# Qi2019KB/UBPL-PoseEstimation

Hardware: AMD Instinct MI355X
Metric: images/sec training step (MT_UBPL, 2-stack HG, 256×256) at 1/2/4/8 GPUs; PCK@0.2 (higher is better)
Workload: dtype fp32; 1 GPU; MT_UBPL train step, 2 students + 2 EMA teachers, 2 views; model=StackedHourglass HG2 (K=16, AvgPool features), global_batch=32, per_gpu_batch=32, input=256x256x3, heatmap=16x64x64, parallelism=dp1

## Files before the change

### include/ubpl_hip.h

```cpp
#ifndef UBPL_HIP_H
#define UBPL_HIP_H
#include <stdint.h>

#ifdef __cplusplus
extern "C" {
#endif

int ubpl_render_heatmaps(const float* kps, float* hm, float* kps_out, int N, int K, int img_h, int img_w,
                         int inp_res, int out_res, float kernel_size, float sigma, float cutoff, void* stream);

int ubpl_heatmap_row_stats(const float* a, int64_t a_sb, int64_t a_ss, const float* t, int64_t t_sb, int64_t t_ss,
                           int64_t t_sm, int M, int B, int S, int K, int HW, float* sq_mean, float* amax,
                           float* tmax, void* stream);
int ubpl_loss_finalize(int kind, const float* sq_mean, const float* amax, const float* tmax, const float* gate,
                       const float* sw, int use_gate, int use_sw, int B, int S, int K, float thr, float* out_sum,
                       int* out_cnt, float* out_score, float* out_w, void* stream);
int ubpl_heatmap_row_grad(const float* a, int64_t a_sb, int64_t a_ss, const float* t, int64_t t_sb, int64_t t_ss,
                          int64_t t_sm, int M, int B, int S, int K, int HW, const float* w, const float* gscale,
                          float extra, float* da, int accumulate, void* stream);

int ubpl_fdl_cov_forward(const float* f1, const float* f2, const float* rowmask, int B, int S, int C, int HW,
                         float* cov, float* mu1, float* mu2, float* out_val, int* out_cnt, void* stream);
int ubpl_fdl_cov_backward(const float* f1, const float* f2, const float* rowmask, const float* cov, const float* mu1,
                          const float* mu2, const int* cnt, const float* gscale, int B, int S, int C, int HW,
// ... 142 lines not shown
int ubpl_upsample2x_add_forward_stats(const float* up, const float* low, int B, int C, int H, int W, float* out,
                                      float* part, void* stream);
int ubpl_bn_forward_stats_maxpool(const float* x, int B, int C, int H, int W, float* y, const float* gamma,
                                  const float* beta, float* rmean, float* rvar, float* mean_out, float* invstd_out,
                                  float* scale, float* shift, const float* pgamma, const float* pbeta, float* prmean,
                                  float* prvar, float* pmean_out, float* pinvstd_out, float* pscale, float* pshift,
                                  float eps, float momentum, double* part, void* stream);
int ubpl_upsample2x_add_forward_bnstats(const float* up, const float* low, int B, int C, int H, int W, float* out,
                                        const float* gamma, const float* beta, float eps, float momentum,
                                        float* rmean, float* rvar, double* part, float* mean_out, float* invstd_out,
                                        float* scale, float* shift, void* stream);
int ubpl_bn_backward_pool(const float* dz, const float* x, int B, int C, int H, int W, const float* gamma,
                          const float* mean, const float* invstd, const float* scale, const float* shift, int relu,
                          double* scratch, const float* part, float* coef, float* dgamma, float* dbeta,
                          const float* add1, const float* pool_dy, const float* add2, float* dx, void* stream);

int ubpl_image_mean_u8(const uint8_t* imgs, int N, int64_t n_per_image, float* out, void* stream);
int ubpl_augment_warp(const uint8_t* imgs, int H, int W, const int* src_idx, const float* mat, const float* noise,
                      const float* img_mean, const float* chan_mean, int V, int Ho, int Wo, float* out, void* stream);

int ubpl_augment_chain(const uint8_t* imgs, int H, int W, const int* geo, const float* cs, const float* noise,
                       const float* img_mean, const float* chan_mean, int V, int Hm, int Wm, float* inter, int Ho,
                       int Wo, float* out, void* stream);

int ubpl_occlude(float* out, int V, int H, int W, const float* bank, const int64_t* off, const int* hw,
                 const int* pastes, const int* view_first, const float* chan_mean, void* stream);

#ifdef __cplusplus
}
#endif
// ... 2 lines not shown
```

### ubpl-poseestimation_amd/csrc/bn_bwd.hip

```cpp
#include "bn.h"

namespace {

__device__ __forceinline__ float fp16_scale_for(float bound) {
    if (!(bound > 0.f) || !isfinite(bound)) return 1.f;
    int e;
    frexpf(bound, &e);
    e = min(max(14 - e, -60), 60);
    return ldexpf(1.f, e);
}

template <bool VEC, bool BOUND>
__global__ void __launch_bounds__(256) bwd_stats_kernel(const float* __restrict__ dz, const float* __restrict__ x,
                                                       int B, int C, int HW, int bper,
                                                       const float* __restrict__ scale,
                                                       const float* __restrict__ shift,
                                                       const float* __restrict__ mean, int relu,
                                                       double* __restrict__ part, unsigned* __restrict__ cnt,
                                                       BwdOut o) {
    __shared__ double red[16];
    __shared__ float redf[16];
    const int c = blockIdx.x, sp = blockIdx.y;
    const int b0 = sp * bper, b1 = min(B, b0 + bper);
    const float sc = scale[c], sh = shift[c], mu = mean[c];
    float s1 = 0.f, s2 = 0.f;
    float mg = 0.f, mx = 0.f;
    if (VEC) {
        const int hw4 = HW >> 2;
        const int n4 = (b1 - b0) * hw4;
        const float4* x4 = reinterpret_cast<const float4*>(x);
        const float4* d4 = reinterpret_cast<const float4*>(dz);
        auto acc1 = [&](float4 xv, float4 g) {
            if (relu) {
                g.x = fmaf(xv.x, sc, sh) > 0.f ? g.x : 0.f;
                g.y = fmaf(xv.y, sc, sh) > 0.f ? g.y : 0.f;
                g.z = fmaf(xv.z, sc, sh) > 0.f ? g.z : 0.f;
                g.w = fmaf(xv.w, sc, sh) > 0.f ? g.w : 0.f;
            }
            s1 += (g.x + g.y) + (g.z + g.w);
            s2 = fmaf(g.x, xv.x - mu, fmaf(g.y, xv.y - mu, fmaf(g.z, xv.z - mu, fmaf(g.w, xv.w - mu, s2))));
            if (BOUND) {
                mg = fmaxf(mg, fmaxf(fmaxf(fabsf(g.x), fabsf(g.y)), fmaxf(fabsf(g.z), fabsf(g.w))));
                mx = fmaxf(mx, fmaxf(fmaxf(fabsf(xv.x - mu), fabsf(xv.y - mu)),
                                     fmaxf(fabsf(xv.z - mu), fabsf(xv.w - mu))));
            }
        };
        auto off_of = [&](int i) {
            const int bb = i / hw4, o4 = i - bb * hw4;
            return ((int64_t)(b0 + bb) * C + c) * hw4 + o4;
        };
        const int st = blockDim.x;
        if (n4 <= 8 * st) {
            float4 xv[8], g[8];
#pragma unroll
            for (int u = 0; u < 8; ++u) {
                const int i = threadIdx.x + u * st;
                if (i < n4) {
                    const int64_t off = off_of(i);
                    xv[u] = x4[off];
                    g[u] = d4[off];
                }
            }
#pragma unroll
            for (int u = 0; u < 8; ++u)
                if (threadIdx.x + u * st < n4) acc1(xv[u], g[u]);
        } else {
            for (int i = threadIdx.x; i < n4; i += st) {
                const int64_t off = off_of(i);
                acc1(x4[off], d4[off]);
            }
        }
    } else {
        const int n = (b1 - b0) * HW;
        for (int i = threadIdx.x; i < n; i += blockDim.x) {
            const int bb = i / HW, o1 = i - bb * HW;
            const int64_t off = ((int64_t)(b0 + bb) * C + c) * HW + o1;
            const float xv = x[off];
            float g = dz[off];
            if (relu && !(fmaf(xv, sc, sh) > 0.f)) g = 0.f;
            s1 += g;
            s2 = fmaf(g, xv - mu, s2);
            if (BOUND) {
                mg = fmaxf(mg, fabsf(g));
                mx = fmaxf(mx, fabsf(xv - mu));
// ... 117 lines not shown

__device__ __forceinline__ void add_pool_grad(float4& v, float4 xv, int64_t off, PoolGeom g, float2 pd) {
    const float4 w = shfl_xor4(xv, 1 << g.lw4);
    const bool bot = (off >> g.lw4) & 1;
    const float4 t = bot ? w : xv, b = bot ? xv : w;
    int a0, a1;
    max4(t.x, t.y, b.x, b.y, a0);
    max4(t.z, t.w, b.z, b.w, a1);
    const int q = bot ? 2 : 0;
    v.x += a0 == q ? pd.x : 0.f;
    v.y += a0 == q + 1 ? pd.x : 0.f;
    v.z += a1 == q ? pd.y : 0.f;
    v.w += a1 == q + 1 ? pd.y : 0.f;
}

struct PoolGrad {
    const float* dy;
    PoolGeom g;
};

template <bool POOL>
__global__ void __launch_bounds__(256) bwd_apply_vec_kernel(const float* dz, const float* __restrict__ x, int C,
                                                           int HW4, int64_t total4, const float* __restrict__ scale,
                                                           const float* __restrict__ shift,
                                                           const float* __restrict__ mean, int relu,
                                                           const float* __restrict__ ca,
                                                           const float* __restrict__ cb,
                                                           const float* __restrict__ cc, const float* add1,
                                                           const float* add2, float* dx, PoolGrad p) {
    const int64_t stride = (int64_t)gridDim.x * blockDim.x;
    for (int64_t i = (int64_t)blockIdx.x * blockDim.x + threadIdx.x; i < total4; i += stride) {
        const int c = (int)((POOL ? i >> p.g.lhw4 : i / HW4) % C);
        const float sc = scale[c], sh = shift[c], mu = mean[c], a = ca[c], b = cb[c], cx = cc[c];
        const float4 xv = reinterpret_cast<const float4*>(x)[i];
        const float4 g = reinterpret_cast<const float4*>(dz)[i];
        float2 pd;
        if (POOL) pd = reinterpret_cast<const float2*>(p.dy)[half_index(i, p.g)];
        float4 v = bwd_one4(g, xv, sc, sh, mu, a, b, cx, relu);
        if (add1) add4(v, reinterpret_cast<const float4*>(add1)[i]);
        if (POOL) add_pool_grad(v, xv, i, p.g, pd);
        if (add2) add4(v, reinterpret_cast<const float4*>(add2)[i]);
        reinterpret_cast<float4*>(dx)[i] = v;
    }
}

template <bool POOL, int U>
__global__ void __launch_bounds__(256) bwd_apply_plane_kernel(const float* dz, const float* __restrict__ x, int C,
                                                             int HW4, const float* __restrict__ scale,
                                                             const float* __restrict__ shift,
                                                             const float* __restrict__ mean, int relu,
                                                             const float* __restrict__ ca,
                                                             const float* __restrict__ cb,
                                                             const float* __restrict__ cc, const float* add1,
                                                             const float* add2, float* dx, PoolGrad p) {
    const int pl = blockIdx.y;
    const int c = pl % C;
    const float sc = scale[c], sh = shift[c], mu = mean[c], a = ca[c], b = cb[c], cx = cc[c];
    const int64_t base = (int64_t)pl * HW4 + blockIdx.x * (256 * U) + threadIdx.x;
    const float4* x4 = reinterpret_cast<const float4*>(x) + base;
    const float4* d4 = reinterpret_cast<const float4*>(dz) + base;
    float4 xv[U], g[U], q1[U], q2[U];
    float2 pd[U];
#pragma unroll
    for (int u = 0; u < U; ++u) {
        xv[u] = x4[u * 256];
        g[u] = d4[u * 256];
        if (POOL) pd[u] = reinterpret_cast<const float2*>(p.dy)[half_index(base + u * 256, p.g)];
        if (add1) q1[u] = reinterpret_cast<const float4*>(add1)[base + u * 256];
        if (add2) q2[u] = reinterpret_cast<const float4*>(add2)[base + u * 256];
    }
#pragma unroll
    for (int u = 0; u < U; ++u) {
        float4 v = bwd_one4(g[u], xv[u], sc, sh, mu, a, b, cx, relu);
        if (add1) add4(v, q1[u]);
        if (POOL) add_pool_grad(v, xv[u], base + u * 256, p.g, pd[u]);
        if (add2) add4(v, q2[u]);
        reinterpret_cast<float4*>(dx)[base + u * 256] = v;
    }
}

__global__ void __launch_bounds__(256) bwd_apply_kernel(const float* dz, const float* __restrict__ x, int C, int HW,
                                                       int64_t total, const float* __restrict__ scale,
                                                       const float* __restrict__ shift,
                                                       const float* __restrict__ mean, int relu,
                                                       const float* __restrict__ ca, const float* __restrict__ cb,
                                                       const float* __restrict__ cc, const float* add1,
                                                       const float* add2, float* dx) {
    const int64_t stride = (int64_t)gridDim.x * blockDim.x;
    for (int64_t i = (int64_t)blockIdx.x * blockDim.x + threadIdx.x; i < total; i += stride) {
        const int c = (int)((i / HW) % C);
// ... 25 lines not shown
    const int64_t HW = (int64_t)H * W;
    const int64_t o = ((int64_t)b * C + 16 * g) * HW + (in ? h * W + w : 0);
    float v[16];
#pragma unroll
    for (int j = 0; j < 16; ++j) {
        const int c = 16 * g + j;
        const float r = bwd_one(dz[o + j * HW], x[o + j * HW], scale[c], shift[c], mean[c], ca[c], cb[c], cc[c], relu);
        v[j] = in ? r : 0.f;
    }
    ubpl::store_psa_row<NP>(v, dst + (((int64_t)(b * G + g) * Hp + hp) * Wp + wq) * 16, plane,
                            NP == 2 ? *dxscale : 1.f);
}

int bwd_stats(const float* dz, const float* x, int B, int C, int HW, const float* gamma, const float* mean,
              const float* invstd, const float* scale, const float* shift, int relu, double* scratch,
              const float* part, float* coef, float* dgamma, float* dbeta, hipStream_t st, bool bound = false) {
    BwdOut o{gamma, invstd, dgamma, dbeta, coef, coef + C, coef + 2 * C, nullptr, nullptr, nullptr};
    if (part != nullptr) {
        if (bound) return (int)hipErrorInvalidValue;
        const int64_t N = (int64_t)B * HW;
        hipLaunchKernelGGL(bn_bwd_finalize_kernel, dim3(C), dim3(FT), 0, st, part, (N + 63) / 64, N, o);
        UBPL_LAUNCH_CHECK();
        return 0;
    }
    if (C > MAXBN || scratch == nullptr) return (int)hipErrorInvalidValue;
    int bper, gs;
    stats_grid(B, C, HW, bper, gs);
    const Scratch s = carve(scratch);
    if (bound) {
        o.bnd = s.bnd;
        o.tcnt = s.tcnt;
        o.dxscale = coef + 3 * C;
    }
    const bool vec = (HW % 4 == 0) && ((((uintptr_t)dz | (uintptr_t)x) & 15) == 0);
    return pick(
        [&](auto VEC, auto BOUND) {
            hipLaunchKernelGGL((bwd_stats_kernel<VEC != 0, BOUND != 0>), dim3(C, gs), dim3(256), 0, st, dz, x, B, C,
                               HW, bper, scale, shift, mean, relu, s.slab, s.cnt, o);
            UBPL_LAUNCH_CHECK();
            return 0;
        },
        among<0, 1>{vec}, among<0, 1>{bound});
}

template <bool POOL>
int launch_apply4(const float* dz, const float* x, int B, int C, int HW, const float* scale, const float* shift,
                  const float* mean, int relu, const float* coef, const float* add1, const float* add2, float* dx,
                  PoolGrad p, hipStream_t st) {
    const float *ca = coef, *cb = coef + C, *cc = coef + 2 * C;
    const int hw4 = HW / 4;
    if (hw4 % 256 != 0 || (int64_t)B * C >= 65536) {
        const int64_t total4 = (int64_t)B * C * hw4;
        hipLaunchKernelGGL(bwd_apply_vec_kernel<POOL>, dim3(grid_ew(total4)), dim3(256), 0, st, dz, x, C, hw4, total4,
                           scale, shift, mean, relu, ca, cb, cc, add1, add2, dx, p);
        UBPL_LAUNCH_CHECK();
        return 0;
    }
    const int u = hw4 % 1024 == 0 ? 4 : (hw4 % 512 == 0 ? 2 : 1);
    return pick(
        [&](auto U) {
            hipLaunchKernelGGL((bwd_apply_plane_kernel<POOL, U>), dim3((unsigned)(hw4 / (256 * U)), (unsigned)(B * C)),
                               dim3(256), 0, st, dz, x, C, hw4, scale, shift, mean, relu, ca, cb, cc, add1, add2, dx,
                               p);
            UBPL_LAUNCH_CHECK();
            return 0;
        },
        among<4, 2, 1>{u});
}

}

UBPL_API int ubpl_bn_backward_partials(const float* dz, const float* x, int B, int C, int HW, const float* scale,
                                       const float* shift, const float* mean, int relu, float* part, void* stream) {
    const int64_t N = (int64_t)B * HW;
    const int64_t np = (N + 63) / 64;
    const bool vec = (HW % 4 == 0) && ((((uintptr_t)dz | (uintptr_t)x) & 15) == 0);
// ... 29 lines not shown
            return 0;
        },
        among<1, 2, 3>{npieces});
}

UBPL_API int ubpl_bn_backward(const float* dz, const float* x, int B, int C, int HW, const float* gamma,
                              const float* mean, const float* invstd, const float* scale, const float* shift,
                              int relu, double* scratch, const float* part, float* coef, float* dgamma,
                              float* dbeta, const float* add1, const float* add2, float* dx, void* stream) {
    hipStream_t st = (hipStream_t)stream;
    const int e = bwd_stats(dz, x, B, C, HW, gamma, mean, invstd, scale, shift, relu, scratch, part, coef, dgamma,
                            dbeta, st);
    if (e) return e;
    const uintptr_t al = (uintptr_t)dz | (uintptr_t)x | (uintptr_t)dx | (uintptr_t)add1 | (uintptr_t)add2;
    if (HW % 4 == 0 && (al & 15) == 0)
        return launch_apply4<false>(dz, x, B, C, HW, scale, shift, mean, relu, coef, add1, add2, dx, PoolGrad{}, st);
    const int64_t total = (int64_t)B * C * HW;
    hipLaunchKernelGGL(bwd_apply_kernel, dim3(grid_ew(total)), dim3(256), 0, st, dz, x, C, HW, total, scale, shift,
                       mean, relu, coef, coef + C, coef + 2 * C, add1, add2, dx);
    UBPL_LAUNCH_CHECK();
    return 0;
}

UBPL_API int ubpl_bn_backward_pool(const float* dz, const float* x, int B, int C, int H, int W, const float* gamma,
                                   const float* mean, const float* invstd, const float* scale, const float* shift,
                                   int relu, double* scratch, const float* part, float* coef, float* dgamma,
                                   float* dbeta, const float* add1, const float* pool_dy, const float* add2,
                                   float* dx, void* stream) {
    const int HW = H * W;
    if (pool_dy == nullptr)
        return ubpl_bn_backward(dz, x, B, C, HW, gamma, mean, invstd, scale, shift, relu, scratch, part, coef, dgamma,
                                dbeta, add1, add2, dx, stream);
    PoolGrad p{pool_dy, {}};
    const uintptr_t al = (uintptr_t)dz | (uintptr_t)x | (uintptr_t)dx | (uintptr_t)add1 | (uintptr_t)add2;
    if (B < 1 || C < 1 || !pool_geom(H, W, p.g) || (al & 15) || (((uintptr_t)pool_dy) & 7))
        return (int)hipErrorInvalidValue;
    hipStream_t st = (hipStream_t)stream;
    const int e = bwd_stats(dz, x, B, C, HW, gamma, mean, invstd, scale, shift, relu, scratch, part, coef, dgamma,
                            dbeta, st);
    if (e) return e;
    return launch_apply4<true>(dz, x, B, C, HW, scale, shift, mean, relu, coef, add1, add2, dx, p, st);
}
```

### ubpl-poseestimation_amd/csrc/pool.hip

```cpp
#include "common.h"

namespace {

int grid_ew(int64_t n) {
    int64_t g = (n + 255) / 256;
    if (g > 8192) g = 8192;
    if (g < 1) g = 1;
    return (int)g;
}

__device__ __forceinline__ void wave_bn_partial(float v, int64_t i0, int C, int P, int64_t np, float* part) {
    const float s = ubpl::wave_sum(v);
    const float d = v - s * (1.f / 64.f);
    const float m2 = ubpl::wave_sum(d * d);
    if ((threadIdx.x & 63) == 0) {
        const int64_t bc = i0 / P;
        const int c = (int)(bc % C);
        const int64_t q = ((bc / C) * P + (i0 - bc * P)) >> 6;
        part[((int64_t)c * np + q) * 2] = s;
        part[((int64_t)c * np + q) * 2 + 1] = m2;
    }
}

template <bool STATS>
// ... 57 lines not shown
__global__ void __launch_bounds__(256) avgpool_fwd_kernel(const float* __restrict__ x, int64_t planes, int H, int W,
                                                         float* __restrict__ y) {
    const int Ho = H >> 1, Wo = W >> 1;
    const int64_t total = planes * Ho * Wo;
    const int64_t stride = (int64_t)gridDim.x * blockDim.x;
    for (int64_t i = (int64_t)blockIdx.x * blockDim.x + threadIdx.x; i < total; i += stride) {
        const int ow = (int)(i % Wo);
        const int64_t t = i / Wo;
        const int oh = (int)(t % Ho);
        const int64_t pl = t / Ho;
        const float* p = x + (pl * H + 2 * oh) * W + 2 * ow;
        y[i] = (((p[0] + p[1]) + p[W]) + p[W + 1]) / 4.f;
    }
}

__global__ void __launch_bounds__(256) avgpool_bwd_kernel(const float* __restrict__ dy, int64_t planes, int H, int W,
                                                         float* __restrict__ dx, int accumulate) {
    const int Ho = H >> 1, Wo = W >> 1;
    const int64_t total = planes * Ho * Wo;
    const int64_t stride = (int64_t)gridDim.x * blockDim.x;
    for (int64_t i = (int64_t)blockIdx.x * blockDim.x + threadIdx.x; i < total; i += stride) {
        const int ow = (int)(i % Wo);
        const int64_t t = i / Wo;
        const int oh = (int)(t % Ho);
        const int64_t pl = t / Ho;
        const int64_t base = (pl * H + 2 * oh) * W + 2 * ow;
        const float g = dy[i] / 4.f;
        const int64_t offs[4] = {0, 1, W, W + 1};
#pragma unroll
        for (int q = 0; q < 4; ++q) {
// ... 71 lines not shown
            const float4 v = reinterpret_cast<const float4*>(x)[src];
            reinterpret_cast<float4*>(y)[i] = make_float4(v.w, v.z, v.y, v.x);
        } else {
            y[i] = x[src];
        }
    }
}

}

UBPL_API int ubpl_fliplr(const float* x, int64_t planes, int H, int W, float* y, void* stream) {
    if (planes < 0 || H < 0 || W < 0 || x == y) return (int)hipErrorInvalidValue;
    const int64_t rows = planes * H;
    if (rows == 0 || W == 0) return 0;
    if ((W % 4) == 0 && ((((uintptr_t)x) | ((uintptr_t)y)) & 15) == 0) {
        hipLaunchKernelGGL(fliplr_kernel<true>, dim3(grid_ew(rows * (W / 4))), dim3(256), 0, (hipStream_t)stream, x,
                           rows, W, y);
    } else {
        hipLaunchKernelGGL(fliplr_kernel<false>, dim3(grid_ew(rows * W)), dim3(256), 0, (hipStream_t)stream, x, rows,
                           W, y);
    }
    UBPL_LAUNCH_CHECK();
    return 0;
}

UBPL_API int ubpl_maxpool2x2_forward(const float* x, int64_t planes, int H, int W, float* y, void* stream) {
    const int64_t n = planes * (H / 2) * (W / 2);
    if (n == 0) return 0;
    hipLaunchKernelGGL(maxpool_fwd_kernel<false>, dim3(grid_ew(n)), dim3(256), 0, (hipStream_t)stream, x, planes, H,
                       W, y, 1, nullptr);
    UBPL_LAUNCH_CHECK();
    return 0;
}

UBPL_API int ubpl_maxpool2x2_forward_stats(const float* x, int B, int C, int H, int W, float* y, float* part,
                                           void* stream) {
    const int64_t planes = (int64_t)B * C;
    if (((H / 2) * (W / 2)) % 64 != 0 || part == nullptr) return (int)hipErrorInvalidValue;
    const int64_t n = planes * (H / 2) * (W / 2);
    if (n == 0) return 0;
    hipLaunchKernelGGL(maxpool_fwd_kernel<true>, dim3(grid_ew(n)), dim3(256), 0, (hipStream_t)stream, x, planes, H,
                       W, y, C, part);
    UBPL_LAUNCH_CHECK();
    return 0;
}

UBPL_API int ubpl_maxpool2x2_backward(const float* x, const float* dy, int64_t planes, int H, int W, float* dx,
                                      int accumulate, void* stream) {
    const int64_t n = planes * (H / 2) * (W / 2);
    if (n == 0) return 0;
    hipLaunchKernelGGL(maxpool_bwd_kernel, dim3(grid_ew(n)), dim3(256), 0, (hipStream_t)stream, x, dy, planes, H, W,
                       dx, accumulate);
    UBPL_LAUNCH_CHECK();
    return 0;
}

UBPL_API int ubpl_avgpool2x2_forward(const float* x, int64_t planes, int H, int W, float* y, void* stream) {
    const int64_t n = planes * (H / 2) * (W / 2);
    if (n == 0) return 0;
    hipLaunchKernelGGL(avgpool_fwd_kernel, dim3(grid_ew(n)), dim3(256), 0, (hipStream_t)stream, x, planes, H, W, y);
    UBPL_LAUNCH_CHECK();
    return 0;
}

UBPL_API int ubpl_avgpool2x2_backward(const float* dy, int64_t planes, int H, int W, float* dx, int accumulate,
                                      void* stream) {
    const int64_t n = planes * (H / 2) * (W / 2);
    if (n == 0) return 0;
    hipLaunchKernelGGL(avgpool_bwd_kernel, dim3(grid_ew(n)), dim3(256), 0, (hipStream_t)stream, dy, planes, H, W, dx,
                       accumulate);
    UBPL_LAUNCH_CHECK();
    return 0;
}

UBPL_API int ubpl_upsample2x_add_forward(const float* up, const float* low, int64_t planes, int H, int W, float* out,
                                         void* stream) {
    const int64_t n = planes * H * W;
    if (n == 0) return 0;
    if ((W % 4) == 0 && ((((uintptr_t)up) | ((uintptr_t)out)) & 15) == 0 && (((uintptr_t)low) & 7) == 0) {
        hipLaunchKernelGGL(upadd_fwd_vec_kernel, dim3(grid_ew(n / 4)), dim3(256), 0, (hipStream_t)stream, up, low, H,
                           W, n / 4, out);
        UBPL_LAUNCH_CHECK();
        return 0;
    }
    hipLaunchKernelGGL(upadd_fwd_kernel<false>, dim3(grid_ew(n)), dim3(256), 0, (hipStream_t)stream, up, low, planes,
                       H, W, out, 1, nullptr);
    UBPL_LAUNCH_CHECK();
    return 0;
}

UBPL_API int ubpl_upsample2x_add_forward_stats(const float* up, const float* low, int B, int C, int H, int W,
                                               float* out, float* part, void* stream) {
    const int64_t planes = (int64_t)B * C;
    if ((H * W) % 64 != 0 || part == nullptr) return (int)hipErrorInvalidValue;
    const int64_t n = planes * H * W;
    if (n == 0) return 0;
    hipLaunchKernelGGL(upadd_fwd_kernel<true>, dim3(grid_ew(n)), dim3(256), 0, (hipStream_t)stream, up, low, planes,
                       H, W, out, C, part);
    UBPL_LAUNCH_CHECK();
    return 0;
}

UBPL_API int ubpl_upsample2x_add_backward(const float* dout, int64_t planes, int H, int W, float* dlow,
                                          int accumulate, void* stream) {
    const int64_t n = planes * (H / 2) * (W / 2);
    if (n == 0) return 0;
    hipLaunchKernelGGL(upadd_bwd_kernel, dim3(grid_ew(n)), dim3(256), 0, (hipStream_t)stream, dout, planes, H, W, dlow,
                       accumulate);
    UBPL_LAUNCH_CHECK();
    return 0;
}

UBPL_API int ubpl_add(const float* a, const float* b, int64_t n, float* out, void* stream) {
    if (n == 0) return 0;
    hipLaunchKernelGGL(add_kernel, dim3(grid_ew(n)), dim3(256), 0, (hipStream_t)stream, a, b, n, out);
    UBPL_LAUNCH_CHECK();
    return 0;
}
```

### ubpl-poseestimation_amd/ubpl_amd/hourglass.py

```python
import math
import os

import torch
from torch import nn

from . import _lib
from . import kernels as Kn

BN_EPS = 1e-5
BN_MOMENTUM = 0.1
_PRODUCER_STATS = os.environ.get("UBPL_PRODUCER_STATS", "0") == "1"
_WGRAD3_64 = os.environ.get("UBPL_WGRAD3_64", "1") != "0"
_WGRAD1_SPLIT = os.environ.get("UBPL_WGRAD1_SPLIT", "1") != "0"
_BWD_EPI = os.environ.get("UBPL_BWD_EPI", "0") == "1"
_STEM_S2D = os.environ.get("UBPL_STEM_S2D", "1") != "0"
_STEM_WGRAD = os.environ.get("UBPL_STEM_WGRAD", "1") != "0"
_FWD_EPI = os.environ.get("UBPL_FWD_EPI", "0") == "1"
_FP16_BWD3 = os.environ.get("UBPL_FP16_BWD3", "1") != "0"
_UPADD_OOP = os.environ.get("UBPL_UPADD_OOP", "0") == "1"
_RELAYOUT_ONCE = os.environ.get("UBPL_RELAYOUT_ONCE", "0") == "1"
_SAVE_LOW3 = os.environ.get("UBPL_SAVE_LOW3", "")
_POOL_FUSE = 0 if (_PRODUCER_STATS or _FWD_EPI or _UPADD_OOP or _SAVE_LOW3) else \
    {"0": 0, "2": 2}.get(os.environ.get("UBPL_POOL_FUSE", "1"), 1)

# ... 410 lines not shown
        x1 = x
        if ex.fuse_ok(x1) and ex.fuse == 2:
            x = ex.bn_maxpool(None, x1, "pre.3.bn1")
            ex.give_coef(x, "pre.3.bn1")
        else:
            part = ex.stat_buffer((x1.shape[0], x1.shape[1], x1.shape[2] // 2, x1.shape[3] // 2))
            x = Kn.maxpool2x2(x1, stat_part=part)
            ex.give_part(x, part)
        ex.save("pre.2", x1)
        x = ex.residual("pre.3", x)
        x = ex.residual("pre.4", x)
        preds, feats = [], []
        for i in range(self.nStack):
            hg = ex.hourglass("hgs.%d.0" % i, 4, x, "features.%d.0.bn1" % i)
            f0 = ex.residual("features.%d.0" % i, hg)
            f = ex.conv_bn_relu("features.%d.1" % i, f0)
            if self.mode != "default" and not frozen:
                feats.append(Kn.avgpool2x2(f) if self.mode == "AvgPool" else Kn.maxpool2x2(f))
            pr = ex.conv("preds.%d.conv" % i, f)
            preds.append(pr)
            if i < self.nStack - 1:
                t = ex.conv("merge_preds.%d.conv.conv" % i, pr, res=x)
                x, part = ex.conv("merge_features.%d.conv.conv" % i, f, res=t, out=t, stats=True)
                ex.give_part(x, part)
            ex.save("stack.%d" % i, (f, pr))
        P = torch.stack(preds, 1)
        Fs = torch.stack(feats, 1) if feats else None
        return P, Fs, ex

    def _backward_impl(self, ex, dpreds, dfeats):
        ex.backward(dpreds, dfeats)


class _HourglassFn(torch.autograd.Function):
    @staticmethod
    def forward(ctx, imgs, anchor, model):
        preds, feats, ex = model._forward_impl(imgs, save=True)
        ctx.ex = ex
        ctx.model = model
        if feats is None:
# ... 144 lines not shown
    def stem(self, imgs):
        if self.ws.pieces in (1, 2, 3) and _STEM_S2D and Kn.stem_s2d_ok(imgs):
            np_ = Kn.backward_pieces(self.ws.pieces)
            ws = self.ws.stem_split(np_)
            xs = Kn.stem_s2d_split(imgs, 2, np_)
            y0 = Kn.conv2d_forward_psa(xs, ws, self.ws.P("pre.0.conv.bias"))
            if self.do_save and _STEM_WGRAD:
                self.saved_split["pre.0.conv"] = xs
        else:
            y0 = self.conv("pre.0.conv", imgs, stride=2)
        sc, sh = self.bn("pre.0.bn", y0)
        x0 = Kn.bn_apply(y0, sc, sh, relu=1)
        self.save("pre.0", (imgs, y0))
        return x0

    def conv_bn_relu(self, p, x):
        y, part = self.conv(p + ".conv", x, stats=True)
        sc, sh = self.bn(p + ".bn", y, part)
        f = Kn.bn_apply(y, sc, sh, relu=1)
        self.save(p, (x, y))
        return f

    def residual(self, p, x):
        cin = x.shape[1]
        cout = self.m._offs[p + ".conv3.conv.weight"][2][0]
        part = self.take_part(x)
        c1 = self.bnc(p + ".bn1")[:2] if self.take_coef(x, p + ".bn1") else self.bn(p + ".bn1", x, part)
        t1, part = self.conv(p + ".conv1.conv", x, pro=c1, stats=True)
        c2 = self.bn(p + ".bn2", t1, part)
        t2, part = self.conv(p + ".conv2.conv", t1, pro=c2, stats=True)
        c3 = self.bn(p + ".bn3", t2, part)
        if cin != cout:
            r = self.conv(p + ".skip_layer.conv", x)
            out, part = self.conv(p + ".conv3.conv", t2, pro=c3, res=r, out=r, stats=True)
        else:
            out, part = self.conv(p + ".conv3.conv", t2, pro=c3, res=x, stats=True)
# ... 34 lines not shown
        if _SAVE_LOW3 == "add":
            self.save(p + ".add_in", (up1.clone(), low3.clone()))
        out = Kn.upsample2x_add(up1, low3, out=up1, stat_part=part)
        if _SAVE_LOW3 == "add":
            self.save(p + ".add_out", out.clone())
        self.give_part(out, part)
        return out

    def _coef(self):
        return self.bcoef if self.bcoef is not None else self.m._ws[("coef", self.B)]

    def G(self, name):
        s, n, shp = self.m._offs[name]
        return self.gbuf[s:s + n].view(shp)

    def bn_bwd(self, name, dz, x, relu, add1=None, add2=None, out=None, part=None, pool_dy=None):
        sc, sh, mu, istd = self.bnc(name)
        if pool_dy is not None:
            return Kn.bn_backward_pool(dz, x, self.m.P(name + ".weight"), mu, istd, sc, sh, relu, self.bpart,
                                       self._coef(), self.G(name + ".weight"), self.G(name + ".bias"), add1=add1,
                                       pool_dy=pool_dy, add2=add2, out=out, part=part)
        return Kn.bn_backward(dz, x, self.m.P(name + ".weight"), mu, istd, sc, sh, relu, self.bpart, self._coef(),
                              self.G(name + ".weight"), self.G(name + ".bias"), add1=add1, add2=add2, out=out,
                              part=part)

    def bn_bwd_split(self, name, dz, x, relu, part=None, pieces=None, grads=True):
        sc, sh, mu, istd = self.bnc(name)
        return Kn.bn_backward_split(dz, x, self.m.P(name + ".weight"), mu, istd, sc, sh, relu, self.bpart,
                                    self._coef(), self.G(name + ".weight") if grads else None,
                                    self.G(name + ".bias") if grads else None,
                                    self.m.bwd_pieces if pieces is None else pieces, 1, part=None if not grads else part)

# ... 87 lines not shown
        dx = self.residual_bwd(p + ".up1", dout)
        Kn.maxpool2x2_backward(x, dpl, dx, accumulate=True)
        if add2 is not None:
            dx = Kn.add(dx, add2, out=dx)
        return dx

    def backward(self, dpreds, dfeats):
        m = self.m
        S = m.nStack
        dpreds = dpreds.contiguous()
        if dfeats is not None:
            dfeats = dfeats.contiguous()
        dxn = None
        for i in reversed(range(S)):
            f, pr = self.saved.get("stack.%d" % i)
            dpi = dpreds[:, i].contiguous()
            if i < S - 1:
                nmf, nmp = "merge_features.%d.conv.conv" % i, "merge_preds.%d.conv.conv" % i
                self.wgrad(nmf, dxn, f, 1)
                self.wgrad(nmp, dxn, pr, 1)
                dpi = self.dgrad(nmp, dxn, res=dpi, out=dpi)
            npd = "preds.%d.conv" % i
            self.wgrad(npd, dpi, f, 1)
            df = self.dgrad(npd, dpi)
            if i < S - 1:
                df = self.dgrad(nmf, dxn, res=df, out=df)
            if dfeats is not None:
                dfi = dfeats[:, i].contiguous()
                if m.mode == "AvgPool":
                    Kn.avgpool2x2_backward(dfi, df, accumulate=True)
                else:
                    Kn.maxpool2x2_backward(f, dfi, df, accumulate=True)
            f0, yf = self.saved.get("features.%d.1" % i)
            d = self.bn_bwd("features.%d.1.bn" % i, df, yf, relu=1)
            self.wgrad("features.%d.1.conv" % i, d, f0, 1)
            d = self.dgrad("features.%d.1.conv" % i, d)
            d = self.residual_bwd("features.%d.0" % i, d)
            dxn = self.hourglass_bwd("hgs.%d.0" % i, 4, d, add2=dxn)
        d = self.residual_bwd("pre.4", dxn)
        d = self.residual_bwd("pre.3", d)
        x1 = self.saved.get("pre.2")
        dx1 = torch.empty_like(x1)
        Kn.maxpool2x2_backward(x1, d, dx1, accumulate=False)
        d = self.residual_bwd("pre.1", dx1)
        imgs, y0 = self.saved.get("pre.0")
        xs = self.saved_split.get("pre.0.conv")
        w0 = m.P("pre.0.conv.weight")
        if xs is not None and m.bwd_pieces in (1, 3) and d.shape[1] % 64 == 0 and d.shape[3] % 16 == 0:
            ys = self.bn_bwd_split("pre.0.bn", d, y0, relu=1)
# ... 25 lines not shown
```

### ubpl-poseestimation_amd/ubpl_amd/kernels.py

```python
import math
import os

import torch

from . import _lib
from ._lib import call

F32 = torch.float32


def _chk(t, name, dtype=F32):
    if t is None:
        return
    _lib.require_gpu(t)
    if t.dtype != dtype:
        raise TypeError("ubpl_amd: %s must be %s, got %s" % (name, dtype, t.dtype))
    if not t.is_contiguous():
        raise ValueError("ubpl_amd: %s must be contiguous" % name)


def render_heatmaps(kps, img_hw, inp_res, out_res, kernel_size=3.0, sigma=1.0, cutoff=0.01, kps_out=None):
    _chk(kps, "kps")
    N, K, _ = kps.shape
    stride = inp_res / out_res
# ... 936 lines not shown
        return bn_backward(dz, x, gamma, mean, invstd, scale, shift, relu, scratch, coef, dgamma, dbeta, add1=add1,
                           add2=add2, out=out, part=part)
    B, C, H, W = _fuse_geometry("bn_backward_pool", x)
    for nm, t in (("dz", dz), ("add1", add1), ("add2", add2), ("out", out)):
        _same_shape(nm, t, x.shape)
    _same_shape("pool_dy", pool_dy, (B, C, H // 2, W // 2))
    _chk(x, "x")
    _chk(dz, "dz")
    _chk(pool_dy, "pool_dy")
    dx = dz if out is None else out
    call("ubpl_bn_backward_pool", dz, x, B, C, H, W, gamma, mean, invstd, scale, shift, int(relu), scratch, part, coef,
         dgamma, dbeta, add1, pool_dy, add2, dx)
    return dx


def image_mean_u8(imgs):
    _chk(imgs, "imgs", torch.uint8)
    out = torch.empty(imgs.shape[0], device=imgs.device, dtype=F32)
    call("ubpl_image_mean_u8", imgs, imgs.shape[0], imgs[0].numel(), out)
    return out


def augment_warp(imgs, src_idx, mat, noise, img_mean, chan_mean, out):
    _chk(imgs, "imgs", torch.uint8)
    _chk(src_idx, "src_idx", torch.int32)
    for t, n in ((mat, "mat"), (noise, "noise"), (img_mean, "img_mean"), (chan_mean, "chan_mean"), (out, "out")):
        _chk(t, n)
    V, _, Ho, Wo = out.shape
    if mat.numel() != 6 * V or noise.numel() != 3 * V or src_idx.numel() != V:
        raise ValueError("augment_warp: per-view tables do not match %d views" % V)
# ... 69 lines not shown
```

Measured before the change: 453.1 images/sec.

## Fold BN+ReLU into avgpool feature path and fuse avgpool grad into BN backward

In AvgPool mode, the features.N.1 BN+ReLU output is no longer materialized. The pooled features come from a fused bn_relu_avgpool kernel, and the downstream convs and wgrads consume the raw conv output through a prologue scale/shift. In backward, the average-pool gradient is added inside the BN backward stats and apply kernels instead of a separate accumulate pass over df. This saves a full-resolution activation write and read plus a separate pooling-gradient kernel, at the cost of recomputing BN/ReLU in the conv prologues.

```diff
diff --git a/include/ubpl_hip.h b/include/ubpl_hip.h
--- a/include/ubpl_hip.h
+++ b/include/ubpl_hip.h
@@ -180,6 +180,12 @@
                           const float* mean, const float* invstd, const float* scale, const float* shift, int relu,
                           double* scratch, const float* part, float* coef, float* dgamma, float* dbeta,
                           const float* add1, const float* pool_dy, const float* add2, float* dx, void* stream);
+int ubpl_bn_relu_avgpool2x2_forward(const float* x, int B, int C, int H, int W, const float* scale,
+                                    const float* shift, float* y, void* stream);
+int ubpl_bn_backward_avgpool(const float* dz, const float* x, int B, int C, int H, int W, const float* gamma,
+                             const float* mean, const float* invstd, const float* scale, const float* shift, int relu,
+                             double* scratch, float* coef, float* dgamma, float* dbeta, const float* pool_dy,
+                             const float* add1, const float* add2, float* dx, void* stream);
 
 int ubpl_image_mean_u8(const uint8_t* imgs, int N, int64_t n_per_image, float* out, void* stream);
 int ubpl_augment_warp(const uint8_t* imgs, int H, int W, const int* src_idx, const float* mat, const float* noise,
diff --git a/ubpl-poseestimation_amd/csrc/bn_bwd.hip b/ubpl-poseestimation_amd/csrc/bn_bwd.hip
--- a/ubpl-poseestimation_amd/csrc/bn_bwd.hip
+++ b/ubpl-poseestimation_amd/csrc/bn_bwd.hip
@@ -10,14 +10,23 @@
     return ldexpf(1.f, e);
 }
 
-template <bool VEC, bool BOUND>
+__device__ __forceinline__ void add_avg_grad(float4& g, float2 l) {
+    const float a = l.x / 4.f, b = l.y / 4.f;
+    g.x += a;
+    g.y += a;
+    g.z += b;
+    g.w += b;
+}
+
+template <bool VEC, bool BOUND, bool AVG = false>
 __global__ void __launch_bounds__(256) bwd_stats_kernel(const float* __restrict__ dz, const float* __restrict__ x,
                                                        int B, int C, int HW, int bper,
                                                        const float* __restrict__ scale,
                                                        const float* __restrict__ shift,
                                                        const float* __restrict__ mean, int relu,
                                                        double* __restrict__ part, unsigned* __restrict__ cnt,
-                                                       BwdOut o) {
+                                                       BwdOut o, const float* __restrict__ dlow, PoolGeom pg) {
+    static_assert(!AVG || (VEC && !BOUND), "the average-pool addend: the float4 path, no bound");
     __shared__ double red[16];
     __shared__ float redf[16];
     const int c = blockIdx.x, sp = blockIdx.y;
@@ -30,6 +39,11 @@
         const int n4 = (b1 - b0) * hw4;
         const float4* x4 = reinterpret_cast<const float4*>(x);
         const float4* d4 = reinterpret_cast<const float4*>(dz);
+        auto dz_at = [&](int64_t off) {
+            float4 g = d4[off];
+            if (AVG) add_avg_grad(g, reinterpret_cast<const float2*>(dlow)[half_index(off, pg)]);
+            return g;
+        };
         auto acc1 = [&](float4 xv, float4 g) {
             if (relu) {
                 g.x = fmaf(xv.x, sc, sh) > 0.f ? g.x : 0.f;
@@ -58,7 +72,7 @@
                 if (i < n4) {
                     const int64_t off = off_of(i);
                     xv[u] = x4[off];
-                    g[u] = d4[off];
+                    g[u] = dz_at(off);
                 }
             }
 #pragma unroll
@@ -67,7 +81,7 @@
         } else {
             for (int i = threadIdx.x; i < n4; i += st) {
                 const int64_t off = off_of(i);
-                acc1(x4[off], d4[off]);
+                acc1(x4[off], dz_at(off));
             }
         }
     } else {
@@ -215,12 +229,14 @@
     v.w += a1 == q + 1 ? pd.y : 0.f;
 }
 
+constexpr int PLAIN = 0, MAXPOOL = 1, AVGPOOL = 2;
+
 struct PoolGrad {
     const float* dy;
     PoolGeom g;
 };
 
-template <bool POOL>
+template <int MODE>
 __global__ void __launch_bounds__(256) bwd_apply_vec_kernel(const float* dz, const float* __restrict__ x, int C,
                                                            int HW4, int64_t total4, const float* __restrict__ scale,
                                                            const float* __restrict__ shift,
@@ -231,21 +247,22 @@
                                                            const float* add2, float* dx, PoolGrad p) {
     const int64_t stride = (int64_t)gridDim.x * blockDim.x;
     for (int64_t i = (int64_t)blockIdx.x * blockDim.x + threadIdx.x; i < total4; i += stride) {
-        const int c = (int)((POOL ? i >> p.g.lhw4 : i / HW4) % C);
+        const int c = (int)((MODE ? i >> p.g.lhw4 : i / HW4) % C);
         const float sc = scale[c], sh = shift[c], mu = mean[c], a = ca[c], b = cb[c], cx = cc[c];
         const float4 xv = reinterpret_cast<const float4*>(x)[i];
-        const float4 g = reinterpret_cast<const float4*>(dz)[i];
+        float4 g = reinterpret_cast<const float4*>(dz)[i];
         float2 pd;
-        if (POOL) pd = reinterpret_cast<const float2*>(p.dy)[half_index(i, p.g)];
+        if (MODE) pd = reinterpret_cast<const float2*>(p.dy)[half_index(i, p.g)];
+        if (MODE == AVGPOOL) add_avg_grad(g, pd);
         float4 v = bwd_one4(g, xv, sc, sh, mu, a, b, cx, relu);
         if (add1) add4(v, reinterpret_cast<const float4*>(add1)[i]);
-        if (POOL) add_pool_grad(v, xv, i, p.g, pd);
+        if (MODE == MAXPOOL) add_pool_grad(v, xv, i, p.g, pd);
         if (add2) add4(v, reinterpret_cast<const float4*>(add2)[i]);
         reinterpret_cast<float4*>(dx)[i] = v;
     }
 }
 
-template <bool POOL, int U>
+template <int MODE, int U>
 __global__ void __launch_bounds__(256) bwd_apply_plane_kernel(const float* dz, const float* __restrict__ x, int C,
                                                              int HW4, const float* __restrict__ scale,
                                                              const float* __restrict__ shift,
@@ -266,15 +283,16 @@
     for (int u = 0; u < U; ++u) {
         xv[u] = x4[u * 256];
         g[u] = d4[u * 256];
-        if (POOL) pd[u] = reinterpret_cast<const float2*>(p.dy)[half_index(base + u * 256, p.g)];
+        if (MODE) pd[u] = reinterpret_cast<const float2*>(p.dy)[half_index(base + u * 256, p.g)];
         if (add1) q1[u] = reinterpret_cast<const float4*>(add1)[base + u * 256];
         if (add2) q2[u] = reinterpret_cast<const float4*>(add2)[base + u * 256];
     }
 #pragma unroll
     for (int u = 0; u < U; ++u) {
+        if (MODE == AVGPOOL) add_avg_grad(g[u], pd[u]);
         float4 v = bwd_one4(g[u], xv[u], sc, sh, mu, a, b, cx, relu);
         if (add1) add4(v, q1[u]);
-        if (POOL) add_pool_grad(v, xv[u], base + u * 256, p.g, pd[u]);
+        if (MODE == MAXPOOL) add_pool_grad(v, xv[u], base + u * 256, p.g, pd[u]);
         if (add2) add4(v, q2[u]);
         reinterpret_cast<float4*>(dx)[base + u * 256] = v;
     }
@@ -330,7 +348,8 @@
 
 int bwd_stats(const float* dz, const float* x, int B, int C, int HW, const float* gamma, const float* mean,
               const float* invstd, const float* scale, const float* shift, int relu, double* scratch,
-              const float* part, float* coef, float* dgamma, float* dbeta, hipStream_t st, bool bound = false) {
+              const float* part, float* coef, float* dgamma, float* dbeta, hipStream_t st, bool bound = false,
+              const PoolGrad* avg = nullptr) {
     BwdOut o{gamma, invstd, dgamma, dbeta, coef, coef + C, coef + 2 * C, nullptr, nullptr, nullptr};
     if (part != nullptr) {
         if (bound) return (int)hipErrorInvalidValue;
@@ -349,17 +368,24 @@
         o.dxscale = coef + 3 * C;
     }
     const bool vec = (HW % 4 == 0) && ((((uintptr_t)dz | (uintptr_t)x) & 15) == 0);
+    if (avg != nullptr) {
+        if (!vec || bound) return (int)hipErrorInvalidValue;
+        hipLaunchKernelGGL((bwd_stats_kernel<true, false, true>), dim3(C, gs), dim3(256), 0, st, dz, x, B, C, HW, bper,
+                           scale, shift, mean, relu, s.slab, s.cnt, o, avg->dy, avg->g);
+        UBPL_LAUNCH_CHECK();
+        return 0;
+    }
     return pick(
         [&](auto VEC, auto BOUND) {
             hipLaunchKernelGGL((bwd_stats_kernel<VEC != 0, BOUND != 0>), dim3(C, gs), dim3(256), 0, st, dz, x, B, C,
-                               HW, bper, scale, shift, mean, relu, s.slab, s.cnt, o);
+                               HW, bper, scale, shift, mean, relu, s.slab, s.cnt, o, nullptr, PoolGeom{});
             UBPL_LAUNCH_CHECK();
             return 0;
         },
         among<0, 1>{vec}, among<0, 1>{bound});
 }
 
-template <bool POOL>
+template <int MODE>
 int launch_apply4(const float* dz, const float* x, int B, int C, int HW, const float* scale, const float* shift,
                   const float* mean, int relu, const float* coef, const float* add1, const float* add2, float* dx,
                   PoolGrad p, hipStream_t st) {
@@ -367,7 +393,7 @@
     const int hw4 = HW / 4;
     if (hw4 % 256 != 0 || (int64_t)B * C >= 65536) {
         const int64_t total4 = (int64_t)B * C * hw4;
-        hipLaunchKernelGGL(bwd_apply_vec_kernel<POOL>, dim3(grid_ew(total4)), dim3(256), 0, st, dz, x, C, hw4, total4,
+        hipLaunchKernelGGL(bwd_apply_vec_kernel<MODE>, dim3(grid_ew(total4)), dim3(256), 0, st, dz, x, C, hw4, total4,
                            scale, shift, mean, relu, ca, cb, cc, add1, add2, dx, p);
         UBPL_LAUNCH_CHECK();
         return 0;
@@ -375,7 +401,7 @@
     const int u = hw4 % 1024 == 0 ? 4 : (hw4 % 512 == 0 ? 2 : 1);
     return pick(
         [&](auto U) {
-            hipLaunchKernelGGL((bwd_apply_plane_kernel<POOL, U>), dim3((unsigned)(hw4 / (256 * U)), (unsigned)(B * C)),
+            hipLaunchKernelGGL((bwd_apply_plane_kernel<MODE, U>), dim3((unsigned)(hw4 / (256 * U)), (unsigned)(B * C)),
                                dim3(256), 0, st, dz, x, C, hw4, scale, shift, mean, relu, ca, cb, cc, add1, add2, dx,
                                p);
             UBPL_LAUNCH_CHECK();
@@ -435,7 +461,7 @@
     if (e) return e;
     const uintptr_t al = (uintptr_t)dz | (uintptr_t)x | (uintptr_t)dx | (uintptr_t)add1 | (uintptr_t)add2;
     if (HW % 4 == 0 && (al & 15) == 0)
-        return launch_apply4<false>(dz, x, B, C, HW, scale, shift, mean, relu, coef, add1, add2, dx, PoolGrad{}, st);
+        return launch_apply4<PLAIN>(dz, x, B, C, HW, scale, shift, mean, relu, coef, add1, add2, dx, PoolGrad{}, st);
     const int64_t total = (int64_t)B * C * HW;
     hipLaunchKernelGGL(bwd_apply_kernel, dim3(grid_ew(total)), dim3(256), 0, st, dz, x, C, HW, total, scale, shift,
                        mean, relu, coef, coef + C, coef + 2 * C, add1, add2, dx);
@@ -460,5 +486,21 @@
     const int e = bwd_stats(dz, x, B, C, HW, gamma, mean, invstd, scale, shift, relu, scratch, part, coef, dgamma,
                             dbeta, st);
     if (e) return e;
-    return launch_apply4<true>(dz, x, B, C, HW, scale, shift, mean, relu, coef, add1, add2, dx, p, st);
-}
+    return launch_apply4<MAXPOOL>(dz, x, B, C, HW, scale, shift, mean, relu, coef, add1, add2, dx, p, st);
+}
+
+UBPL_API int ubpl_bn_backward_avgpool(const float* dz, const float* x, int B, int C, int H, int W,
+                                      const float* gamma, const float* mean, const float* invstd,
+                                      const float* scale, const float* shift, int relu, double* scratch, float* coef,
+                                      float* dgamma, float* dbeta, const float* pool_dy, const float* add1,
+                                      const float* add2, float* dx, void* stream) {
+    PoolGrad p{pool_dy, {}};
+    const uintptr_t al = (uintptr_t)dz | (uintptr_t)x | (uintptr_t)dx | (uintptr_t)add1 | (uintptr_t)add2;
+    if (B < 1 || C < 1 || pool_dy == nullptr || !pool_geom(H, W, p.g) || (al & 15) || (((uintptr_t)pool_dy) & 7))
+        return (int)hipErrorInvalidValue;
+    hipStream_t st = (hipStream_t)stream;
+    const int e = bwd_stats(dz, x, B, C, H * W, gamma, mean, invstd, scale, shift, relu, scratch, nullptr, coef,
+                            dgamma, dbeta, st, false, &p);
+    if (e) return e;
+    return launch_apply4<AVGPOOL>(dz, x, B, C, H * W, scale, shift, mean, relu, coef, add1, add2, dx, p, st);
+}
diff --git a/ubpl-poseestimation_amd/csrc/pool.hip b/ubpl-poseestimation_amd/csrc/pool.hip
--- a/ubpl-poseestimation_amd/csrc/pool.hip
+++ b/ubpl-poseestimation_amd/csrc/pool.hip
@@ -1,8 +1,8 @@
-#include "common.h"
+#include "bn.h"
 
 namespace {
 
-int grid_ew(int64_t n) {
+int grid_pool(int64_t n) {
     int64_t g = (n + 255) / 256;
     if (g > 8192) g = 8192;
     if (g < 1) g = 1;
@@ -95,6 +95,27 @@
     }
 }
 
+__global__ void __launch_bounds__(256) bn_relu_avgpool_kernel(const float* __restrict__ x,
+                                                             const float* __restrict__ scale,
+                                                             const float* __restrict__ shift, int C, PoolGeom g,
+                                                             int64_t total2, float* __restrict__ y) {
+    const int64_t stride = (int64_t)gridDim.x * blockDim.x;
+    const int w4 = 1 << g.lw4;
+    for (int64_t i = (int64_t)blockIdx.x * blockDim.x + threadIdx.x; i < total2; i += stride) {
+        const int64_t pl = i >> (g.lhw4 - 1);
+        const int o2 = (int)(i & ((1 << (g.lhw4 - 1)) - 1));
+        const int c = (int)(pl % C);
+        const float sc = scale[c], sh = shift[c];
+        const int64_t top = (pl << g.lhw4) + (((o2 >> g.lw4) << 1) << g.lw4) + (o2 & (w4 - 1));
+        const float4 t = reinterpret_cast<const float4*>(x)[top];
+        const float4 b = reinterpret_cast<const float4*>(x)[top + w4];
+        auto act = [&](float v) { return fmaxf(fmaf(v, sc, sh), 0.f); };
+        reinterpret_cast<float2*>(y)[i] =
+            make_float2((((act(t.x) + act(t.y)) + act(b.x)) + act(b.y)) / 4.f,
+                        (((act(t.z) + act(t.w)) + act(b.z)) + act(b.w)) / 4.f);
+    }
+}
+
 __global__ void __launch_bounds__(256) avgpool_bwd_kernel(const float* __restrict__ dy, int64_t planes, int H, int W,
                                                          float* __restrict__ dx, int accumulate) {
     const int Ho = H >> 1, Wo = W >> 1;
@@ -196,10 +217,10 @@
     const int64_t rows = planes * H;
     if (rows == 0 || W == 0) return 0;
     if ((W % 4) == 0 && ((((uintptr_t)x) | ((uintptr_t)y)) & 15) == 0) {
-        hipLaunchKernelGGL(fliplr_kernel<true>, dim3(grid_ew(rows * (W / 4))), dim3(256), 0, (hipStream_t)stream, x,
+        hipLaunchKernelGGL(fliplr_kernel<true>, dim3(grid_pool(rows * (W / 4))), dim3(256), 0, (hipStream_t)stream, x,
                            rows, W, y);
     } else {
-        hipLaunchKernelGGL(fliplr_kernel<false>, dim3(grid_ew(rows * W)), dim3(256), 0, (hipStream_t)stream, x, rows,
+        hipLaunchKernelGGL(fliplr_kernel<false>, dim3(grid_pool(rows * W)), dim3(256), 0, (hipStream_t)stream, x, rows,
                            W, y);
     }
     UBPL_LAUNCH_CHECK();
@@ -209,7 +230,7 @@
 UBPL_API int ubpl_maxpool2x2_forward(const float* x, int64_t planes, int H, int W, float* y, void* stream) {
     const int64_t n = planes * (H / 2) * (W / 2);
     if (n == 0) return 0;
-    hipLaunchKernelGGL(maxpool_fwd_kernel<false>, dim3(grid_ew(n)), dim3(256), 0, (hipStream_t)stream, x, planes, H,
+    hipLaunchKernelGGL(maxpool_fwd_kernel<false>, dim3(grid_pool(n)), dim3(256), 0, (hipStream_t)stream, x, planes, H,
                        W, y, 1, nullptr);
     UBPL_LAUNCH_CHECK();
     return 0;
@@ -221,7 +242,7 @@
     if (((H / 2) * (W / 2)) % 64 != 0 || part == nullptr) return (int)hipErrorInvalidValue;
     const int64_t n = planes * (H / 2) * (W / 2);
     if (n == 0) return 0;
-    hipLaunchKernelGGL(maxpool_fwd_kernel<true>, dim3(grid_ew(n)), dim3(256), 0, (hipStream_t)stream, x, planes, H,
+    hipLaunchKernelGGL(maxpool_fwd_kernel<true>, dim3(grid_pool(n)), dim3(256), 0, (hipStream_t)stream, x, planes, H,
                        W, y, C, part);
     UBPL_LAUNCH_CHECK();
     return 0;
@@ -231,7 +252,7 @@
                                       int accumulate, void* stream) {
     const int64_t n = planes * (H / 2) * (W / 2);
     if (n == 0) return 0;
-    hipLaunchKernelGGL(maxpool_bwd_kernel, dim3(grid_ew(n)), dim3(256), 0, (hipStream_t)stream, x, dy, planes, H, W,
+    hipLaunchKernelGGL(maxpool_bwd_kernel, dim3(grid_pool(n)), dim3(256), 0, (hipStream_t)stream, x, dy, planes, H, W,
                        dx, accumulate);
     UBPL_LAUNCH_CHECK();
     return 0;
@@ -240,7 +261,20 @@
 UBPL_API int ubpl_avgpool2x2_forward(const float* x, int64_t planes, int H, int W, float* y, void* stream) {
     const int64_t n = planes * (H / 2) * (W / 2);
     if (n == 0) return 0;
-    hipLaunchKernelGGL(avgpool_fwd_kernel, dim3(grid_ew(n)), dim3(256), 0, (hipStream_t)stream, x, planes, H, W, y);
+    hipLaunchKernelGGL(avgpool_fwd_kernel, dim3(grid_pool(n)), dim3(256), 0, (hipStream_t)stream, x, planes, H, W, y);
+    UBPL_LAUNCH_CHECK();
+    return 0;
+}
+
+UBPL_API int ubpl_bn_relu_avgpool2x2_forward(const float* x, int B, int C, int H, int W, const float* scale,
+                                             const float* shift, float* y, void* stream) {
+    PoolGeom g;
+    if (B < 1 || C < 1 || !pool_geom(H, W, g) || (((uintptr_t)x) & 15) || (((uintptr_t)y) & 7) || scale == nullptr ||
+        shift == nullptr)
+        return (int)hipErrorInvalidValue;
+    const int64_t total2 = ((int64_t)B * C) << (g.lhw4 - 1);
+    hipLaunchKernelGGL(bn_relu_avgpool_kernel, dim3(grid_pool(total2)), dim3(256), 0, (hipStream_t)stream, x, scale,
+                       shift, C, g, total2, y);
     UBPL_LAUNCH_CHECK();
     return 0;
 }
@@ -249,7 +283,7 @@
                                       void* stream) {
     const int64_t n = planes * (H / 2) * (W / 2);
     if (n == 0) return 0;
-    hipLaunchKernelGGL(avgpool_bwd_kernel, dim3(grid_ew(n)), dim3(256), 0, (hipStream_t)stream, dy, planes, H, W, dx,
+    hipLaunchKernelGGL(avgpool_bwd_kernel, dim3(grid_pool(n)), dim3(256), 0, (hipStream_t)stream, dy, planes, H, W, dx,
                        accumulate);
     UBPL_LAUNCH_CHECK();
     return 0;
@@ -260,12 +294,12 @@
     const int64_t n = planes * H * W;
     if (n == 0) return 0;
     if ((W % 4) == 0 && ((((uintptr_t)up) | ((uintptr_t)out)) & 15) == 0 && (((uintptr_t)low) & 7) == 0) {
-        hipLaunchKernelGGL(upadd_fwd_vec_kernel, dim3(grid_ew(n / 4)), dim3(256), 0, (hipStream_t)stream, up, low, H,
+        hipLaunchKernelGGL(upadd_fwd_vec_kernel, dim3(grid_pool(n / 4)), dim3(256), 0, (hipStream_t)stream, up, low, H,
                            W, n / 4, out);
         UBPL_LAUNCH_CHECK();
         return 0;
     }
-    hipLaunchKernelGGL(upadd_fwd_kernel<false>, dim3(grid_ew(n)), dim3(256), 0, (hipStream_t)stream, up, low, planes,
+    hipLaunchKernelGGL(upadd_fwd_kernel<false>, dim3(grid_pool(n)), dim3(256), 0, (hipStream_t)stream, up, low, planes,
                        H, W, out, 1, nullptr);
     UBPL_LAUNCH_CHECK();
     return 0;
@@ -277,7 +311,7 @@
     if ((H * W) % 64 != 0 || part == nullptr) return (int)hipErrorInvalidValue;
     const int64_t n = planes * H * W;
     if (n == 0) return 0;
-    hipLaunchKernelGGL(upadd_fwd_kernel<true>, dim3(grid_ew(n)), dim3(256), 0, (hipStream_t)stream, up, low, planes,
+    hipLaunchKernelGGL(upadd_fwd_kernel<true>, dim3(grid_pool(n)), dim3(256), 0, (hipStream_t)stream, up, low, planes,
                        H, W, out, C, part);
     UBPL_LAUNCH_CHECK();
     return 0;
@@ -287,7 +321,7 @@
                                           int accumulate, void* stream) {
     const int64_t n = planes * (H / 2) * (W / 2);
     if (n == 0) return 0;
-    hipLaunchKernelGGL(upadd_bwd_kernel, dim3(grid_ew(n)), dim3(256), 0, (hipStream_t)stream, dout, planes, H, W, dlow,
+    hipLaunchKernelGGL(upadd_bwd_kernel, dim3(grid_pool(n)), dim3(256), 0, (hipStream_t)stream, dout, planes, H, W, dlow,
                        accumulate);
     UBPL_LAUNCH_CHECK();
     return 0;
@@ -295,7 +329,7 @@
 
 UBPL_API int ubpl_add(const float* a, const float* b, int64_t n, float* out, void* stream) {
     if (n == 0) return 0;
-    hipLaunchKernelGGL(add_kernel, dim3(grid_ew(n)), dim3(256), 0, (hipStream_t)stream, a, b, n, out);
-    UBPL_LAUNCH_CHECK();
-    return 0;
-}
+    hipLaunchKernelGGL(add_kernel, dim3(grid_pool(n)), dim3(256), 0, (hipStream_t)stream, a, b, n, out);
+    UBPL_LAUNCH_CHECK();
+    return 0;
+}
diff --git a/ubpl-poseestimation_amd/ubpl_amd/hourglass.py b/ubpl-poseestimation_amd/ubpl_amd/hourglass.py
--- a/ubpl-poseestimation_amd/ubpl_amd/hourglass.py
+++ b/ubpl-poseestimation_amd/ubpl_amd/hourglass.py
@@ -448,16 +448,18 @@
         for i in range(self.nStack):
             hg = ex.hourglass("hgs.%d.0" % i, 4, x, "features.%d.0.bn1" % i)
             f0 = ex.residual("features.%d.0" % i, hg)
-            f = ex.conv_bn_relu("features.%d.1" % i, f0)
-            if self.mode != "default" and not frozen:
+            f, fpro = ex.conv_bn_relu("features.%d.1" % i, f0, fold=self.mode == "AvgPool")
+            if fpro is not None:
+                feats.append(Kn.bn_relu_avgpool2x2(f, *fpro))
+            elif self.mode != "default" and not frozen:
                 feats.append(Kn.avgpool2x2(f) if self.mode == "AvgPool" else Kn.maxpool2x2(f))
-            pr = ex.conv("preds.%d.conv" % i, f)
+            pr = ex.conv("preds.%d.conv" % i, f, pro=fpro)
             preds.append(pr)
             if i < self.nStack - 1:
                 t = ex.conv("merge_preds.%d.conv.conv" % i, pr, res=x)
-                x, part = ex.conv("merge_features.%d.conv.conv" % i, f, res=t, out=t, stats=True)
+                x, part = ex.conv("merge_features.%d.conv.conv" % i, f, pro=fpro, res=t, out=t, stats=True)
                 ex.give_part(x, part)
-            ex.save("stack.%d" % i, (f, pr))
+            ex.save("stack.%d" % i, (None if fpro is not None else f, pr))
         P = torch.stack(preds, 1)
         Fs = torch.stack(feats, 1) if feats else None
         return P, Fs, ex
@@ -632,12 +634,13 @@
         self.save("pre.0", (imgs, y0))
         return x0
 
-    def conv_bn_relu(self, p, x):
+    def conv_bn_relu(self, p, x, fold=False):
         y, part = self.conv(p + ".conv", x, stats=True)
         sc, sh = self.bn(p + ".bn", y, part)
-        f = Kn.bn_apply(y, sc, sh, relu=1)
         self.save(p, (x, y))
-        return f
+        if fold and self.fuse_ok(y):
+            return y, (sc, sh)
+        return Kn.bn_apply(y, sc, sh, relu=1), None
 
     def residual(self, p, x):
         cin = x.shape[1]
@@ -702,8 +705,12 @@
         s, n, shp = self.m._offs[name]
         return self.gbuf[s:s + n].view(shp)
 
-    def bn_bwd(self, name, dz, x, relu, add1=None, add2=None, out=None, part=None, pool_dy=None):
+    def bn_bwd(self, name, dz, x, relu, add1=None, add2=None, out=None, part=None, pool_dy=None, avg_dy=None):
         sc, sh, mu, istd = self.bnc(name)
+        if avg_dy is not None:
+            return Kn.bn_backward_avgpool(dz, x, self.m.P(name + ".weight"), mu, istd, sc, sh, relu, self.bpart,
+                                          self._coef(), self.G(name + ".weight"), self.G(name + ".bias"), avg_dy,
+                                          add1=add1, add2=add2, out=out)
         if pool_dy is not None:
             return Kn.bn_backward_pool(dz, x, self.m.P(name + ".weight"), mu, istd, sc, sh, relu, self.bpart,
                                        self._coef(), self.G(name + ".weight"), self.G(name + ".bias"), add1=add1,
@@ -821,25 +828,32 @@
         dxn = None
         for i in reversed(range(S)):
             f, pr = self.saved.get("stack.%d" % i)
+            f0, yf = self.saved.get("features.%d.1" % i)
+            fpro = None
+            if f is None:
+                f, fpro = yf, self.bnc("features.%d.1.bn" % i)[:2]
             dpi = dpreds[:, i].contiguous()
             if i < S - 1:
                 nmf, nmp = "merge_features.%d.conv.conv" % i, "merge_preds.%d.conv.conv" % i
-                self.wgrad(nmf, dxn, f, 1)
+                self.wgrad(nmf, dxn, f, 1, pro=fpro)
                 self.wgrad(nmp, dxn, pr, 1)
                 dpi = self.dgrad(nmp, dxn, res=dpi, out=dpi)
             npd = "preds.%d.conv" % i
-            self.wgrad(npd, dpi, f, 1)
+            self.wgrad(npd, dpi, f, 1, pro=fpro)
             df = self.dgrad(npd, dpi)
             if i < S - 1:
                 df = self.dgrad(nmf, dxn, res=df, out=df)
+            avg_dy = None
             if dfeats is not None:
                 dfi = dfeats[:, i].contiguous()
-                if m.mode == "AvgPool":
+                if m.mode != "AvgPool":
+                    Kn.maxpool2x2_backward(f, dfi, df, accumulate=True)
+                elif _POOL_FUSE and Kn.pool_fuse_ok(yf.shape[2], yf.shape[3], yf.shape[1], yf, df) \
+                        and dfi.data_ptr() % 8 == 0:
+                    avg_dy = dfi
+                else:
                     Kn.avgpool2x2_backward(dfi, df, accumulate=True)
-                else:
-                    Kn.maxpool2x2_backward(f, dfi, df, accumulate=True)
-            f0, yf = self.saved.get("features.%d.1" % i)
-            d = self.bn_bwd("features.%d.1.bn" % i, df, yf, relu=1)
+            d = self.bn_bwd("features.%d.1.bn" % i, df, yf, relu=1, avg_dy=avg_dy)
             self.wgrad("features.%d.1.conv" % i, d, f0, 1)
             d = self.dgrad("features.%d.1.conv" % i, d)
             d = self.residual_bwd("features.%d.0" % i, d)
diff --git a/ubpl-poseestimation_amd/ubpl_amd/kernels.py b/ubpl-poseestimation_amd/ubpl_amd/kernels.py
--- a/ubpl-poseestimation_amd/ubpl_amd/kernels.py
+++ b/ubpl-poseestimation_amd/ubpl_amd/kernels.py
@@ -974,6 +974,42 @@
     return dx
 
 
+def bn_relu_avgpool2x2(x, scale, shift, out=None):
+    if x.dim() != 4:
+        raise ValueError("ubpl_amd: bn_relu_avgpool2x2 takes a [B,C,H,W] tensor, got shape %s" % (tuple(x.shape),))
+    B, C, H, W = x.shape
+    _same_shape("scale", scale, (C,))
+    _same_shape("shift", shift, (C,))
+    _same_shape("out", out, (B, C, H // 2, W // 2))
+    if B < 1 or not pool_fuse_ok(H, W, C, x) or (out is not None and out.data_ptr() % 8):
+        return avgpool2x2(bn_apply(x, scale, shift, relu=1), out=out)
+    _chk(x, "x")
+    y = torch.empty((B, C, H // 2, W // 2), device=x.device, dtype=F32) if out is None else out
+    call("ubpl_bn_relu_avgpool2x2_forward", x, B, C, H, W, scale, shift, y)
+    return y
+
+
+def bn_backward_avgpool(dz, x, gamma, mean, invstd, scale, shift, relu, scratch, coef, dgamma, dbeta, pool_dy,
+                        add1=None, add2=None, out=None):
+    if x.dim() != 4:
+        raise ValueError("ubpl_amd: bn_backward_avgpool takes a [B,C,H,W] tensor, got shape %s" % (tuple(x.shape),))
+    B, C, H, W = x.shape
+    for nm, t in (("dz", dz), ("add1", add1), ("add2", add2), ("out", out)):
+        _same_shape(nm, t, x.shape)
+    _same_shape("pool_dy", pool_dy, (B, C, H // 2, W // 2))
+    if B < 1 or not pool_fuse_ok(H, W, C, x, dz, add1, add2, out) or pool_dy.data_ptr() % 8:
+        avgpool2x2_backward(pool_dy, dz, accumulate=True)
+        return bn_backward(dz, x, gamma, mean, invstd, scale, shift, relu, scratch, coef, dgamma, dbeta, add1=add1,
+                           add2=add2, out=out)
+    _chk(x, "x")
+    _chk(dz, "dz")
+    _chk(pool_dy, "pool_dy")
+    dx = dz if out is None else out
+    call("ubpl_bn_backward_avgpool", dz, x, B, C, H, W, gamma, mean, invstd, scale, shift, int(relu), scratch, coef,
+         dgamma, dbeta, pool_dy, add1, add2, dx)
+    return dx
+
+
 def image_mean_u8(imgs):
     _chk(imgs, "imgs", torch.uint8)
     out = torch.empty(imgs.shape[0], device=imgs.device, dtype=F32)
```

Measured after the change: 452.5 images/sec. About the same (-0.1%).
